# plai-group/latent-flexible-video-diffusion-modeling

Hardware: NVIDIA B200
Metric: denoiser frame-steps/sec (sampling) (higher is better)
Workload: dtype bf16

## Files before the change

latent-flexible-video-diffusion-modeling_b200/csrc/attn_temporal_tc.cu:

```cuda
#include "tc_common.cuh"
#include <mutex>

namespace fdm {

struct TtParams {
  const float* mask;
  __nv_bfloat16* b2;
  __nv_bfloat16* b3;
  __nv_bfloat16* P;
  __nv_bfloat16* out;
  float* attn_mean;
  int B, T, HW, C, F, heads;
  int TS;
  int Tn;
  int cf;
  int rows;
  int tmem_cols;
  float scale_log2e;
};

__device__ __forceinline__ uint64_t tt_desc_mn(uint32_t saddr) {
  uint64_t d = 0;
  d |= (uint64_t)((saddr & 0x3FFFF) >> 4);
  d |= (uint64_t)1 << 16;
  d |= (uint64_t)(1024 >> 4) << 32;
  d |= (uint64_t)1 << 46;
  d |= (uint64_t)2 << 61;
  return d;
}

__device__ __forceinline__ void tt_bulk_load(void* dst, const void* src, uint32_t bytes, uint64_t* bar) {
  asm volatile("cp.async.bulk.shared::cluster.global.mbarrier::complete_tx::bytes [%0], [%1], %2, [%3];"
               ::"r"(smem_u32(dst)), "l"(src), "r"(bytes), "r"(smem_u32(bar)) : "memory");
}

__device__ __forceinline__ uint32_t tt_pack(float a, float b) {
  __nv_bfloat162 v = __floats2bfloat162_rn(a, b);
  return *reinterpret_cast<uint32_t*>(&v);
}

template <class RowPtr>
__device__ __forceinline__ void tt_store_rows8(uint8_t* stage, int lane, const uint4 (&w)[4], RowPtr row_ptr, int np) {
#pragma unroll
  for (int q = 0; q < 4; ++q) *reinterpret_cast<uint4*>(stage + lane * 80 + q * 16) = w[q];
  __syncwarp();
  for (int idx = lane; idx < 32 * np; idx += 32) {
    const int row = idx / np, pc = idx - row * np;
    uint8_t* d = row_ptr(row);
    if (d != nullptr) *reinterpret_cast<uint2*>(d + pc * 8) = *reinterpret_cast<const uint2*>(stage + row * 80 + pc * 8);
  }
  __syncwarp();
}

__global__ void __launch_bounds__(128) rpe_bias_kernel(const __grid_constant__ CUtensorMap tq, const __grid_constant__ CUtensorMap trk,
                                                       const __grid_constant__ CUtensorMap trq, const TtParams p) {
  extern __shared__ uint8_t smem_raw[];
  uint8_t* smem = reinterpret_cast<uint8_t*>((reinterpret_cast<uintptr_t>(smem_raw) + 1023) & ~uintptr_t(1023));
  __shared__ __align__(8) uint64_t bar_load, bar_d;
  __shared__ uint32_t tmem_slot;
  const int tid = threadIdx.x, warp = tid >> 5;
  const int px0 = blockIdx.x * 128, j = blockIdx.y, bh = blockIdx.z;
  const int b = bh / p.heads, h = bh - b * p.heads;
  const int F = p.F, C = p.C, Tn = p.Tn;
  const int rtile = Tn * 128;
  uint8_t* q_s = smem;
  uint8_t* k_s = q_s + p.cf * 16384;
  uint8_t* rk_s = k_s + p.cf * 16384;
  uint8_t* rq_s = rk_s + p.cf * rtile;
  if (tid == 0) {
    asm volatile("prefetch.tensormap [%0];" ::"l"(&tq) : "memory");
    asm volatile("prefetch.tensormap [%0];" ::"l"(&trk) : "memory");
    asm volatile("prefetch.tensormap [%0];" ::"l"(&trq) : "memory");
    mbar_init(&bar_load, 1);
    mbar_init(&bar_d, 1);
    asm volatile("fence.mbarrier_init.release.cluster;" ::: "memory");
  }
  if (warp == 1) {
    asm volatile("tcgen05.alloc.cta_group::1.sync.aligned.shared::cta.b32 [%0], %1;" ::"r"(smem_u32(&tmem_slot)), "r"(p.tmem_cols));
    asm volatile("tcgen05.relinquish_alloc_permit.cta_group::1.sync.aligned;");
  }
  tcgen05_fence_before();
  __syncthreads();
  tcgen05_fence_after();
  const uint32_t tmem = tmem_slot;
  pdl_wait();
  if (tid == 0) {
    mbar_expect_tx(&bar_load, (uint32_t)(p.cf * (2 * p.rows * 128 + 2 * rtile)));
    for (int c = 0; c < p.cf; ++c) {
      const int ch = h * F + c * 64;
      tma_load_3d(q_s + c * 16384, &tq, &bar_load, ch, px0, b * p.T + j);
      tma_load_3d(k_s + c * 16384, &tq, &bar_load, C + ch, px0, b * p.T + j);
      tma_load_3d(rk_s + c * rtile, &trk, &bar_load, ch, 0, b * p.T + j);
      tma_load_3d(rq_s + c * rtile, &trq, &bar_load, ch, 0, b * p.T + j);
    }
    mbar_wait(&bar_load, 0);
    tcgen05_fence_after();
    const uint32_t idesc = make_idesc(Tn);
    const int ksteps = F / 16;
    for (int ks = 0; ks < ksteps; ++ks) {
      const int c = ks >> 2, kk = ks & 3;
      umma_bf16(tmem, make_smem_desc(smem_u32(q_s + c * 16384)) + 2 * kk, make_smem_desc(smem_u32(rk_s + c * rtile)) + 2 * kk, idesc, ks != 0);
    }
    for (int ks = 0; ks < ksteps; ++ks) {
      const int c = ks >> 2, kk = ks & 3;
      umma_bf16(tmem + Tn, make_smem_desc(smem_u32(k_s + c * 16384)) + 2 * kk, make_smem_desc(smem_u32(rq_s + c * rtile)) + 2 * kk, idesc, ks != 0);
    }
    umma_commit(&bar_d);
  }
  __syncwarp();
  mbar_wait(&bar_d, 0);
  tcgen05_fence_after();
  const uint32_t trow = tmem + ((uint32_t)(warp * 32) << 16);
  const int px = px0 + tid;
  const bool ok = tid < p.rows && px < p.HW;
  uint8_t* stage = smem + warp * 2560;
  const int lane = tid & 31;
  const int r0 = warp * 32;
  (void)ok;
  (void)px;
  for (int c0 = 0; c0 < Tn && c0 < p.TS; c0 += 32) {
    uint32_t v2[32], v3[32];
    {
      uint32_t a[16];
      tmem_ld_32x32b_x16(trow + c0, a);
#pragma unroll
      for (int k = 0; k < 16; ++k) v2[k] = a[k];
      tmem_ld_32x32b_x16(trow + Tn + c0, a);
#pragma unroll
      for (int k = 0; k < 16; ++k) v3[k] = a[k];
      if (c0 + 16 < Tn) {
        tmem_ld_32x32b_x16(trow + c0 + 16, a);
#pragma unroll
        for (int k = 0; k < 16; ++k) v2[16 + k] = a[k];
        tmem_ld_32x32b_x16(trow + Tn + c0 + 16, a);
#pragma unroll
        for (int k = 0; k < 16; ++k) v3[16 + k] = a[k];
      } else {
#pragma unroll
        for (int k = 0; k < 16; ++k) v2[16 + k] = v3[16 + k] = 0u;
      }
    }
    const int np = min(8, (p.TS - c0) / 4);
    auto rowp = [&](__nv_bfloat16* base, int r) -> uint8_t* {
      const int rr = r0 + r;
      if (rr >= p.rows || px0 + rr >= p.HW) return nullptr;
      return reinterpret_cast<uint8_t*>(base + (((size_t)bh * p.HW + px0 + rr) * p.T + j) * p.TS + c0);
    };
    uint4 w[4];
#pragma unroll
    for (int k = 0; k < 4; ++k)
      w[k] = make_uint4(tt_pack(__uint_as_float(v2[8 * k]), __uint_as_float(v2[8 * k + 1])), tt_pack(__uint_as_float(v2[8 * k + 2]), __uint_as_float(v2[8 * k + 3])),
                        tt_pack(__uint_as_float(v2[8 * k + 4]), __uint_as_float(v2[8 * k + 5])), tt_pack(__uint_as_float(v2[8 * k + 6]), __uint_as_float(v2[8 * k + 7])));
    if ((p.TS & 7) == 0) warp_store_rows64(stage, lane, w, [&](int r) { return rowp(p.b2, r); }, np >> 1);
    else tt_store_rows8(stage, lane, w, [&](int r) { return rowp(p.b2, r); }, np);
#pragma unroll
    for (int k = 0; k < 4; ++k)
      w[k] = make_uint4(tt_pack(__uint_as_float(v3[8 * k]), __uint_as_float(v3[8 * k + 1])), tt_pack(__uint_as_float(v3[8 * k + 2]), __uint_as_float(v3[8 * k + 3])),
                        tt_pack(__uint_as_float(v3[8 * k + 4]), __uint_as_float(v3[8 * k + 5])), tt_pack(__uint_as_float(v3[8 * k + 6]), __uint_as_float(v3[8 * k + 7])));
    if ((p.TS & 7) == 0) warp_store_rows64(stage, lane, w, [&](int r) { return rowp(p.b3, r); }, np >> 1);
    else tt_store_rows8(stage, lane, w, [&](int r) { return rowp(p.b3, r); }, np);
  }
  tcgen05_fence_before();
  __syncthreads();
  if (warp == 1) {
    tcgen05_fence_after();
    asm volatile("tcgen05.dealloc.cta_group::1.sync.aligned.b32 %0, %1;" ::"r"(tmem), "r"(p.tmem_cols));
  }
}

template <int TP>
__global__ void __launch_bounds__(128) attn_rows_kernel(const __grid_constant__ CUtensorMap tq4, const TtParams p) {
  constexpr int PL = 128 / TP;
  constexpr int W = TP < 32 ? 32 : TP;
  extern __shared__ uint8_t smem_raw[];
  uint8_t* smem = reinterpret_cast<uint8_t*>((reinterpret_cast<uintptr_t>(smem_raw) + 1023) & ~uintptr_t(1023));
  __shared__ __align__(8) uint64_t bar_load, bar_s, bar_o;
  __shared__ uint32_t tmem_slot;
  const int tid = threadIdx.x, warp = tid >> 5;
  const int px0 = blockIdx.x * PL, h = blockIdx.y, b = blockIdx.z;
  const int T = p.T, F = p.F, C = p.C, HW = p.HW;
  uint8_t* v_s = smem;
  uint8_t* q_s = v_s + p.cf * 16384;
  uint8_t* k_s = q_s + p.cf * 16384;
  uint8_t* p_s = q_s;
  if (tid == 0) {
    asm volatile("prefetch.tensormap [%0];" ::"l"(&tq4) : "memory");
    mbar_init(&bar_load, 1);
    mbar_init(&bar_s, 1);
    mbar_init(&bar_o, 1);
    asm volatile("fence.mbarrier_init.release.cluster;" ::: "memory");
  }
  if (warp == 1) {
    asm volatile("tcgen05.alloc.cta_group::1.sync.aligned.shared::cta.b32 [%0], %1;" ::"r"(smem_u32(&tmem_slot)), "r"(128));
    asm volatile("tcgen05.relinquish_alloc_permit.cta_group::1.sync.aligned;");
  }
  tcgen05_fence_before();
  __syncthreads();
  tcgen05_fence_after();
  const uint32_t tmem = tmem_slot;
  pdl_wait();
  const int bh = b * p.heads + h;
  const int TS = p.TS;
  __nv_bfloat16* b2_s = reinterpret_cast<__nv_bfloat16*>(smem + p.cf * 3 * 16384);
  __nv_bfloat16* b3_s = b2_s + PL * T * TS;
  if (tid == 0) {
    const uint32_t bias_bytes = (uint32_t)(PL * T * TS * sizeof(__nv_bfloat16));
    mbar_expect_tx(&bar_load, (uint32_t)(p.cf * 3 * 16384) + 2 * bias_bytes);
    for (int c = 0; c < p.cf; ++c) {
      const int ch = h * F + c * 64;
      tma_load_4d(q_s + c * 16384, &tq4, &bar_load, ch, 0, px0, b);
      tma_load_4d(k_s + c * 16384, &tq4, &bar_load, C + ch, 0, px0, b);
      tma_load_4d(v_s + c * 16384, &tq4, &bar_load, 2 * C + ch, 0, px0, b);
    }
    const size_t blk = ((size_t)bh * HW + px0) * T * TS;
    tt_bulk_load(b2_s, p.b2 + blk, bias_bytes, &bar_load);
    tt_bulk_load(b3_s, p.b3 + blk, bias_bytes, &bar_load);
    mbar_wait(&bar_load, 0);
    tcgen05_fence_after();
    const uint32_t idesc = make_idesc(128);
    const int ksteps = F / 16;
    for (int ks = 0; ks < ksteps; ++ks) {
      const int c = ks >> 2, kk = ks & 3;
      umma_bf16(tmem, make_smem_desc(smem_u32(q_s + c * 16384)) + 2 * kk, make_smem_desc(smem_u32(k_s + c * 16384)) + 2 * kk, idesc, ks != 0);
    }
    umma_commit(&bar_s);
  }
  __syncwarp();
  const int pl = tid / TP, t = tid - pl * TP;
  const int px = px0 + pl;
  const bool valid = t < T && px < HW;
  const int sub = TP < 32 ? (pl % (32 / TP)) : 0;
  const int col0 = (tid / W) * W;
  unsigned long long gbits = ~0ull;
  if (p.mask != nullptr) {
    const int lane = tid & 31;
    const float* maskb = p.mask + (size_t)b * T;
    const unsigned lo = __ballot_sync(0xffffffffu, lane < T && __ldg(maskb + lane) > 0.5f);
    const unsigned hi = __ballot_sync(0xffffffffu, lane + 32 < T && __ldg(maskb + lane + 32) > 0.5f);
    gbits = ((unsigned long long)hi << 32) | lo;
  }
  const bool grp = valid ? ((gbits >> t) & 1ull) != 0 : true;
  mbar_wait(&bar_load, 0);
  float bias[W];
  {
    float bt[TP];
    const __nv_bfloat16* b2r = b2_s + (size_t)(pl * T + (valid ? t : 0)) * TS;
    const __nv_bfloat16* b3col = b3_s + (size_t)pl * T * TS + (valid ? t : 0);
    auto fin = [&](int s, uint32_t bits) {
      const bool okj = valid && s < T && ((((gbits >> s) & 1ull) != 0) == grp);
      bt[s] = okj ? __uint_as_float(bits) + __bfloat162float(b3col[(size_t)(s < T ? s : 0) * TS]) : -INFINITY;
    };
    if ((TS & 7) == 0) {
#pragma unroll
      for (int k = 0; k < TP / 8; ++k) {
        uint4 r = make_uint4(0u, 0u, 0u, 0u);
        if (valid && 8 * k < T) r = reinterpret_cast<const uint4*>(b2r)[k];
        fin(8 * k, r.x << 16); fin(8 * k + 1, r.x & 0xffff0000u); fin(8 * k + 2, r.y << 16); fin(8 * k + 3, r.y & 0xffff0000u);
        fin(8 * k + 4, r.z << 16); fin(8 * k + 5, r.z & 0xffff0000u); fin(8 * k + 6, r.w << 16); fin(8 * k + 7, r.w & 0xffff0000u);
      }
    } else {
#pragma unroll
      for (int k = 0; k < TP / 4; ++k) {
        uint2 r = make_uint2(0u, 0u);
        if (valid && 4 * k < T) r = reinterpret_cast<const uint2*>(b2r)[k];
        fin(4 * k, r.x << 16); fin(4 * k + 1, r.x & 0xffff0000u); fin(4 * k + 2, r.y << 16); fin(4 * k + 3, r.y & 0xffff0000u);
      }
    }
#pragma unroll
    for (int j = 0; j < W; ++j) {
      const bool own = TP >= 32 ? true : ((j / TP) == sub);
      bias[j] = own ? bt[j % TP] : -INFINITY;
    }
  }
  __syncwarp();
  mbar_wait(&bar_s, 0);
  tcgen05_fence_after();

  const uint32_t trow = tmem + ((uint32_t)(warp * 32) << 16);
  float e[W];
  float mx = -INFINITY;
#pragma unroll
  for (int c = 0; c < W; c += 32) {
    uint32_t v[32];
    tmem_ld_32x32b_x32(trow + col0 + c, v);
#pragma unroll
    for (int j = 0; j < 32; ++j) {
      e[c + j] = (__uint_as_float(v[j]) + bias[c + j]) * p.scale_log2e;
      mx = fmaxf(mx, e[c + j]);
    }
  }
  float sum = 0.f;
#pragma unroll
  for (int j = 0; j < W; ++j) {
    e[j] = valid ? exp2f(e[j] - mx) : 0.f;
    sum += e[j];
  }
  const float inv = valid ? 1.f / sum : 0.f;
#pragma unroll
  for (int j = 0; j < W; ++j) e[j] *= inv;
  {
    const int sw = tid & 7;
    const int gp0 = col0 >> 3;
#pragma unroll
    for (int gp = 0; gp < 16; ++gp) {
      uint8_t* dst = p_s + (gp >> 3) * 16384 + tid * 128 + (((gp & 7) ^ sw) << 4);
      if (gp < gp0 || gp >= gp0 + W / 8) *reinterpret_cast<uint4*>(dst) = make_uint4(0u, 0u, 0u, 0u);
    }
#pragma unroll
    for (int q = 0; q < W / 8; ++q) {
      const int gp = gp0 + q;
      uint8_t* dst = p_s + (gp >> 3) * 16384 + tid * 128 + (((gp & 7) ^ sw) << 4);
      *reinterpret_cast<uint4*>(dst) = make_uint4(tt_pack(e[8 * q], e[8 * q + 1]), tt_pack(e[8 * q + 2], e[8 * q + 3]),
                                                  tt_pack(e[8 * q + 4], e[8 * q + 5]), tt_pack(e[8 * q + 6], e[8 * q + 7]));
    }
  }
  fence_proxy_async_smem();
  tcgen05_fence_before();
  __syncthreads();
  if (tid == 0) {
    tcgen05_fence_after();
    for (int c = 0; c < p.cf; ++c) {
      const int nf = min(64, F - c * 64);
      const uint32_t idesc = make_idesc(nf, 1);
      for (int ks = 0; ks < 8; ++ks)
        umma_bf16(tmem + c * 64, make_smem_desc(smem_u32(p_s + (ks >> 2) * 16384)) + 2 * (ks & 3),
                  tt_desc_mn(smem_u32(v_s + c * 16384 + ks * 2048)), idesc, ks != 0);
    }
    umma_commit(&bar_o);
  }
  const int lane = tid & 31;
  if (p.attn_mean != nullptr && valid) {
    float* arow = p.attn_mean + (((size_t)b * HW + px) * T + t) * T;
    const float hw_ = 1.f / (float)p.heads;
#pragma unroll
    for (int j = 0; j < W; ++j) {
      const bool own = TP >= 32 ? true : ((j / TP) == sub);
      if (own && (j % TP) < T) atomicAdd(arow + (j % TP), e[j] * hw_);
    }
  }
  {
    const int k = lane & 7;
#pragma unroll
    for (int i = 0; i < 8; ++i) {
      const int r = warp * 32 + i * 4 + (lane >> 3);
      const int rpl = r / TP, rt = r - rpl * TP;
      if (rt < T && px0 + rpl < HW) {
        uint4 val = make_uint4(0u, 0u, 0u, 0u);
        if (8 * k < TP) {
          const int gp = ((rpl * TP) >> 3) + k;
          val = *reinterpret_cast<const uint4*>(p_s + (gp >> 3) * 16384 + r * 128 + (((gp & 7) ^ (r & 7)) << 4));
        }
        *reinterpret_cast<uint4*>(reinterpret_cast<uint8_t*>(p.P + (((size_t)bh * HW + px0 + rpl) * T + rt) * 64) + k * 16) = val;
      }
    }
  }
  __syncwarp();
  mbar_wait(&bar_o, 0);
  tcgen05_fence_after();
  {
    uint8_t* stage = p_s + warp * 4096;
    for (int f = 0; f < F; f += 32) {
      uint32_t v[32];
      const bool two = f + 16 < F;
      {
        uint32_t a[16];
        tmem_ld_32x32b_x16(trow + f, a);
#pragma unroll
        for (int j = 0; j < 16; ++j) v[j] = a[j];
        if (two) {
          tmem_ld_32x32b_x16(trow + f + 16, a);
#pragma unroll
          for (int j = 0; j < 16; ++j) v[16 + j] = a[j];
        } else {
#pragma unroll
          for (int j = 0; j < 16; ++j) v[16 + j] = 0u;
        }
      }
      uint4 w[4];
#pragma unroll
      for (int k = 0; k < 4; ++k)
        w[k] = make_uint4(tt_pack(__uint_as_float(v[8 * k]), __uint_as_float(v[8 * k + 1])), tt_pack(__uint_as_float(v[8 * k + 2]), __uint_as_float(v[8 * k + 3])),
                          tt_pack(__uint_as_float(v[8 * k + 4]), __uint_as_float(v[8 * k + 5])), tt_pack(__uint_as_float(v[8 * k + 6]), __uint_as_float(v[8 * k + 7])));
      warp_store_rows64(stage, lane, w, [&](int rr) -> uint8_t* {
        const int r = warp * 32 + rr;
        const int rpl = r / TP, rt = r - rpl * TP;
        if (rt >= T || px0 + rpl >= HW) return nullptr;
        return reinterpret_cast<uint8_t*>(p.out + ((size_t)(b * T + rt) * HW + px0 + rpl) * C + h * F + f);
      }, two ? 4 : 2);
    }
  }
  tcgen05_fence_before();
  __syncthreads();
  if (warp == 1) {
    tcgen05_fence_after();
    asm volatile("tcgen05.dealloc.cta_group::1.sync.aligned.b32 %0, %1;" ::"r"(tmem), "r"(128));
  }
}

__global__ void __launch_bounds__(128) rpe_pv_kernel(const __grid_constant__ CUtensorMap tp4, const __grid_constant__ CUtensorMap trv,
                                                     const __grid_constant__ CUtensorMap to, const TtParams p) {
  extern __shared__ uint8_t smem_raw[];
  uint8_t* smem = reinterpret_cast<uint8_t*>((reinterpret_cast<uintptr_t>(smem_raw) + 1023) & ~uintptr_t(1023));
  __shared__ __align__(8) uint64_t bar_load, bar_d;
  __shared__ uint32_t tmem_slot;
  const int tid = threadIdx.x, warp = tid >> 5;
  const int px0 = blockIdx.x * 128, t = blockIdx.y, bh = blockIdx.z;
  const int b = bh / p.heads, h = bh - b * p.heads;
  const int F = p.F, Tn = p.Tn;
  const int rtile = Tn * 128;
  uint8_t* p_s = smem;
  uint8_t* rv_s = p_s + 16384;
  __nv_bfloat16* o_s = reinterpret_cast<__nv_bfloat16*>(rv_s + p.cf * rtile);
  if (tid == 0) {
    asm volatile("prefetch.tensormap [%0];" ::"l"(&tp4) : "memory");
    asm volatile("prefetch.tensormap [%0];" ::"l"(&trv) : "memory");
    asm volatile("prefetch.tensormap [%0];" ::"l"(&to) : "memory");
    mbar_init(&bar_load, 1);
    mbar_init(&bar_d, 1);
    asm volatile("fence.mbarrier_init.release.cluster;" ::: "memory");
  }
  if (warp == 1) {
    asm volatile("tcgen05.alloc.cta_group::1.sync.aligned.shared::cta.b32 [%0], %1;" ::"r"(smem_u32(&tmem_slot)), "r"(p.tmem_cols));
    asm volatile("tcgen05.relinquish_alloc_permit.cta_group::1.sync.aligned;");
  }
  tcgen05_fence_before();
  __syncthreads();
  tcgen05_fence_after();
  const uint32_t tmem = tmem_slot;
  pdl_wait();
  if (tid == 0) {
    mbar_expect_tx(&bar_load, (uint32_t)(p.rows * 128 + p.cf * rtile + p.rows * F * 2));
    tma_load_4d(p_s, &tp4, &bar_load, 0, t, px0, bh);
    tma_load_3d(o_s, &to, &bar_load, h * F, px0, b * p.T + t);
    for (int c = 0; c < p.cf; ++c) tma_load_3d(rv_s + c * rtile, &trv, &bar_load, h * F + c * 64, 0, b * p.T + t);
    mbar_wait(&bar_load, 0);
    tcgen05_fence_after();
    for (int c = 0; c < p.cf; ++c) {
      const int nf = min(64, F - c * 64);
      const uint32_t idesc = make_idesc(nf, 1);
      for (int ks = 0; ks < Tn / 16; ++ks)
        umma_bf16(tmem + c * 64, make_smem_desc(smem_u32(p_s)) + 2 * ks, tt_desc_mn(smem_u32(rv_s + c * rtile + ks * 2048)), idesc, ks != 0);
    }
    umma_commit(&bar_d);
  }
  __syncwarp();
  mbar_wait(&bar_d, 0);
  tcgen05_fence_after();
  const uint32_t trow = tmem + ((uint32_t)(warp * 32) << 16);
  const int px = px0 + tid;
  const bool ok = tid < p.rows && px < p.HW;
  const __nv_bfloat16* osrc = o_s + (size_t)(ok ? tid : 0) * F;
  uint8_t* stage = p_s + warp * 2560;
  const int lane = tid & 31;
  for (int f = 0; f < F; f += 32) {
    uint32_t v[32];
    const bool two = f + 16 < F;
    {
      uint32_t a[16];
      tmem_ld_32x32b_x16(trow + f, a);
#pragma unroll
      for (int j = 0; j < 16; ++j) v[j] = a[j];
      if (two) {
        tmem_ld_32x32b_x16(trow + f + 16, a);
#pragma unroll
        for (int j = 0; j < 16; ++j) v[16 + j] = a[j];
      } else {
#pragma unroll
        for (int j = 0; j < 16; ++j) v[16 + j] = 0u;
      }
    }
    uint4 w[4];
#pragma unroll
    for (int k = 0; k < 4; ++k) {
      uint4 o = make_uint4(0u, 0u, 0u, 0u);
      if (ok && (k < 2 || two)) o = *reinterpret_cast<const uint4*>(osrc + f + 8 * k);
      const uint32_t ow[4] = {o.x, o.y, o.z, o.w};
      uint32_t r[4];
#pragma unroll
      for (int q = 0; q < 4; ++q)
        r[q] = tt_pack(__uint_as_float(ow[q] << 16) + __uint_as_float(v[8 * k + 2 * q]),
                       __uint_as_float(ow[q] & 0xffff0000u) + __uint_as_float(v[8 * k + 2 * q + 1]));
      w[k] = make_uint4(r[0], r[1], r[2], r[3]);
    }
    warp_store_rows64(stage, lane, w, [&](int rr) -> uint8_t* {
      const int r = warp * 32 + rr;
      if (r >= p.rows || px0 + r >= p.HW) return nullptr;
      return reinterpret_cast<uint8_t*>(p.out + ((size_t)(b * p.T + t) * p.HW + px0 + r) * p.C + h * F + f);
    }, two ? 4 : 2);
  }
  tcgen05_fence_before();
  __syncthreads();
  if (warp == 1) {
    tcgen05_fence_after();
    asm volatile("tcgen05.dealloc.cta_group::1.sync.aligned.b32 %0, %1;" ::"r"(tmem), "r"(p.tmem_cols));
  }
}

static int tt_pow2(int v, int lo) {
  int r = lo;
  while (r < v) r <<= 1;
  return r;
}
static inline int tt_round_up(int v, int m) { return (v + m - 1) / m * m; }
int tt_row_stride(int T) {
  int t16 = tt_round_up(T, 8);
  if (((t16 / 8) & 1) == 0) t16 += 8;
  int t8 = tt_round_up(T, 4);
  if (((t8 / 4) & 1) == 0) t8 += 4;
  return t16 <= t8 ? t16 : t8;
}

static bool tt_shape_ok(const fdm_attn_temporal_args* a) {
  if (a->qkv_dtype != FDM_BF16 || a->out_dtype != FDM_BF16) return false;
  if (a->heads <= 0 || a->C % a->heads) return false;
  const int F = a->C / a->heads;
  if (F % 16 || F > 128 || a->C % 8) return false;
  if (a->T < 1 || a->T > 64) return false;
  const int TP = a->T <= 8 ? 8 : (a->T <= 16 ? 16 : (a->T <= 32 ? 32 : 64));
  if (a->HW % (128 / TP)) return false;
  return true;
}

size_t attn_temporal_tc_workspace(const fdm_attn_temporal_args* a) {
  if (!tt_shape_ok(a)) return 0;
  const size_t rows = (size_t)a->B * a->heads * a->HW * a->T;
  const size_t TS = tt_row_stride(a->T);
  return 2 * rows * TS * sizeof(__nv_bfloat16) + rows * 64 * sizeof(__nv_bfloat16);
}

template <typename Kern>
static int tt_set_smem(Kern k, int bytes) {
  cudaError_t e = cudaFuncSetAttribute(k, cudaFuncAttributeMaxDynamicSharedMemorySize, bytes);
  if (e != cudaSuccess) {
    set_last_error(e);
    return FDM_ERR_CUDA;
  }
  return FDM_OK;
}

static bool tt_encode(CUtensorMap* m, const void* ptr, int rank, const cuuint64_t* dims, const cuuint64_t* strides, const cuuint32_t* box) {
  EncodeTiledFn enc = get_tensormap_encoder();
  if (!enc) return false;
  cuuint32_t estr[4] = {1, 1, 1, 1};
  return enc(m, CU_TENSOR_MAP_DATA_TYPE_BFLOAT16, rank, const_cast<void*>(ptr), dims, strides, box, estr, CU_TENSOR_MAP_INTERLEAVE_NONE,
             CU_TENSOR_MAP_SWIZZLE_128B, CU_TENSOR_MAP_L2_PROMOTION_L2_128B, CU_TENSOR_MAP_FLOAT_OOB_FILL_NONE) == CUDA_SUCCESS;
}

int attn_temporal_tc_launch(const fdm_attn_temporal_args* a, cudaStream_t st) {
  if (!tt_shape_ok(a) || !a->Rq_op || !a->Rk_op || !a->Rv_op || !a->workspace) return FDM_ERR_UNSUPPORTED;
  const size_t need = attn_temporal_tc_workspace(a);
  FDM_REQUIRE((size_t)a->workspace_bytes >= need, FDM_ERR_BAD_ARG);
  const int B = a->B, T = a->T, HW = a->HW, C = a->C, heads = a->heads, F = C / heads;
  TtParams p;
  p.mask = a->mask;
  p.B = B; p.T = T; p.HW = HW; p.C = C; p.F = F; p.heads = heads;
  p.TS = tt_row_stride(T);
  p.Tn = tt_round_up(T, 16);
  p.cf = (F + 63) / 64;
  p.rows = HW < 128 ? HW : 128;
  p.scale_log2e = 1.4426950408889634f / sqrtf((float)F);
  const size_t rows = (size_t)B * heads * HW * T;
  p.b2 = reinterpret_cast<__nv_bfloat16*>(a->workspace);
  p.b3 = p.b2 + rows * p.TS;
  p.P = reinterpret_cast<__nv_bfloat16*>(p.b3 + rows * p.TS);
  p.out = reinterpret_cast<__nv_bfloat16*>(a->out);
  p.attn_mean = a->attn_mean;
  const int TP = T <= 8 ? 8 : (T <= 16 ? 16 : (T <= 32 ? 32 : 64));
  const int PL = 128 / TP;

  CUtensorMap tq3, tq4, trq, trk, trv, tp4;
  {
    cuuint64_t dims[3] = {(cuuint64_t)3 * C, (cuuint64_t)HW, (cuuint64_t)B * T};
    cuuint64_t strides[2] = {(cuuint64_t)3 * C * 2, (cuuint64_t)HW * 3 * C * 2};
    cuuint32_t box[3] = {64, (cuuint32_t)p.rows, 1};
    FDM_REQUIRE(tt_encode(&tq3, a->qkv, 3, dims, strides, box), FDM_ERR_UNSUPPORTED);
  }
  {
    cuuint64_t dims[4] = {(cuuint64_t)3 * C, (cuuint64_t)T, (cuuint64_t)HW, (cuuint64_t)B};
    cuuint64_t strides[3] = {(cuuint64_t)HW * 3 * C * 2, (cuuint64_t)3 * C * 2, (cuuint64_t)T * HW * 3 * C * 2};
    cuuint32_t box[4] = {64, (cuuint32_t)TP, (cuuint32_t)PL, 1};
    FDM_REQUIRE(tt_encode(&tq4, a->qkv, 4, dims, strides, box), FDM_ERR_UNSUPPORTED);
  }
  {
    cuuint64_t dims[3] = {(cuuint64_t)C, (cuuint64_t)T, (cuuint64_t)B * T};
    cuuint64_t strides[2] = {(cuuint64_t)C * 2, (cuuint64_t)T * C * 2};
    cuuint32_t box[3] = {64, (cuuint32_t)p.Tn, 1};
    FDM_REQUIRE(tt_encode(&trq, a->Rq_op, 3, dims, strides, box) && tt_encode(&trk, a->Rk_op, 3, dims, strides, box) &&
                    tt_encode(&trv, a->Rv_op, 3, dims, strides, box), FDM_ERR_UNSUPPORTED);
  }
  {
    cuuint64_t dims[4] = {64, (cuuint64_t)T, (cuuint64_t)HW, (cuuint64_t)B * heads};
    cuuint64_t strides[3] = {128, (cuuint64_t)T * 128, (cuuint64_t)HW * T * 128};
    cuuint32_t box[4] = {64, 1, (cuuint32_t)p.rows, 1};
    FDM_REQUIRE(tt_encode(&tp4, p.P, 4, dims, strides, box), FDM_ERR_UNSUPPORTED);
  }
  CUtensorMap to;
  {
    EncodeTiledFn enc = get_tensormap_encoder();
    cuuint64_t dims[3] = {(cuuint64_t)C, (cuuint64_t)HW, (cuuint64_t)B * T};
    cuuint64_t strides[2] = {(cuuint64_t)C * 2, (cuuint64_t)HW * C * 2};
    cuuint32_t box[3] = {(cuuint32_t)F, (cuuint32_t)p.rows, 1};
    cuuint32_t estr[3] = {1, 1, 1};
    FDM_REQUIRE(enc != nullptr && enc(&to, CU_TENSOR_MAP_DATA_TYPE_BFLOAT16, 3, a->out, dims, strides, box, estr, CU_TENSOR_MAP_INTERLEAVE_NONE,
                                      CU_TENSOR_MAP_SWIZZLE_NONE, CU_TENSOR_MAP_L2_PROMOTION_L2_128B,
                                      CU_TENSOR_MAP_FLOAT_OOB_FILL_NONE) == CUDA_SUCCESS, FDM_ERR_UNSUPPORTED);
  }
  const int smem1 = p.cf * (2 * 16384 + 2 * p.Tn * 128) + 1024;
  const int smem2 = p.cf * 3 * 16384 + 2 * PL * T * p.TS * (int)sizeof(__nv_bfloat16) + 1024;
  const int smem3 = 16384 + p.cf * p.Tn * 128 + p.rows * F * 2 + 1024;
  static std::once_flag once;
  static int attr_rc = FDM_OK;
  std::call_once(once, [] {
    int rc = tt_set_smem(rpe_bias_kernel, 100 * 1024);
    if (rc == FDM_OK) rc = tt_set_smem(attn_rows_kernel<8>, 200 * 1024);
    if (rc == FDM_OK) rc = tt_set_smem(attn_rows_kernel<16>, 200 * 1024);
    if (rc == FDM_OK) rc = tt_set_smem(attn_rows_kernel<32>, 200 * 1024);
    if (rc == FDM_OK) rc = tt_set_smem(attn_rows_kernel<64>, 200 * 1024);
    if (rc == FDM_OK) rc = tt_set_smem(rpe_pv_kernel, 100 * 1024);
    attr_rc = rc;
  });
  if (attr_rc != FDM_OK) return attr_rc;
  FDM_REQUIRE(smem1 <= 100 * 1024 && smem2 <= 200 * 1024 && smem3 <= 100 * 1024, FDM_ERR_UNSUPPORTED);

  TtParams p1 = p;
  p1.tmem_cols = tt_pow2(2 * p.Tn, 32);
  dim3 gridA((HW + 127) / 128, T, B * heads);
  fdm::launch(rpe_bias_kernel, gridA, dim3(128), smem1, st, tq3, trk, trq, p1);
  int rc = check_launch();
  if (rc != FDM_OK) return rc;
  dim3 gridB(HW / PL, heads, B);
  switch (TP) {
    case 8: fdm::launch(attn_rows_kernel<8>, gridB, dim3(128), smem2, st, tq4, p); break;
    case 16: fdm::launch(attn_rows_kernel<16>, gridB, dim3(128), smem2, st, tq4, p); break;
    case 32: fdm::launch(attn_rows_kernel<32>, gridB, dim3(128), smem2, st, tq4, p); break;
    default: fdm::launch(attn_rows_kernel<64>, gridB, dim3(128), smem2, st, tq4, p); break;
  }
  rc = check_launch();
  if (rc != FDM_OK) return rc;
  TtParams p3 = p;
  p3.tmem_cols = tt_pow2(F, 32);
  fdm::launch(rpe_pv_kernel, gridA, dim3(128), smem3, st, tp4, trv, to, p3);
  return check_launch();
}

}
```

Measured before the change: 94730.

## Pack temporal attention rows densely by T instead of padded power-of-two tiles

```diff
diff --git a/latent-flexible-video-diffusion-modeling_b200/csrc/attn_temporal_tc.cu b/latent-flexible-video-diffusion-modeling_b200/csrc/attn_temporal_tc.cu
--- a/latent-flexible-video-diffusion-modeling_b200/csrc/attn_temporal_tc.cu
+++ b/latent-flexible-video-diffusion-modeling_b200/csrc/attn_temporal_tc.cu
@@ -1,4 +1,5 @@
 #include "tc_common.cuh"
+#include <algorithm>
 #include <mutex>
 
 namespace fdm {
@@ -17,6 +18,11 @@
   int rows;
   int tmem_cols;
   float scale_log2e;
+  int v_stride;
+  int qk_row;
+  int qk_chunks;
+  int qk_stride;
+  int bias_cap;
 };
 
 __device__ __forceinline__ uint64_t tt_desc_mn(uint32_t saddr) {
@@ -26,6 +32,16 @@
   d |= (uint64_t)(1024 >> 4) << 32;
   d |= (uint64_t)1 << 46;
   d |= (uint64_t)2 << 61;
+  return d;
+}
+
+__device__ __forceinline__ uint64_t tt_desc_k64(uint32_t saddr) {
+  uint64_t d = 0;
+  d |= (uint64_t)((saddr & 0x3FFFF) >> 4);
+  d |= (uint64_t)1 << 16;
+  d |= (uint64_t)(512 >> 4) << 32;
+  d |= (uint64_t)1 << 46;
+  d |= (uint64_t)4 << 61;
   return d;
 }
 
@@ -168,23 +184,28 @@
   }
 }
 
-template <int TP>
-__global__ void __launch_bounds__(128) attn_rows_kernel(const __grid_constant__ CUtensorMap tq4, const TtParams p) {
-  constexpr int PL = 128 / TP;
-  constexpr int W = TP < 32 ? 32 : TP;
+template <int NC>
+__global__ void __launch_bounds__(128, NC <= 4 ? 4 : 2) attn_rows_kernel(const __grid_constant__ CUtensorMap tqk4, const __grid_constant__ CUtensorMap tv4,
+                                                        const TtParams p) {
   extern __shared__ uint8_t smem_raw[];
   uint8_t* smem = reinterpret_cast<uint8_t*>((reinterpret_cast<uintptr_t>(smem_raw) + 1023) & ~uintptr_t(1023));
   __shared__ __align__(8) uint64_t bar_load, bar_s, bar_o;
   __shared__ uint32_t tmem_slot;
-  const int tid = threadIdx.x, warp = tid >> 5;
+  const int tid = threadIdx.x, warp = tid >> 5, lane = tid & 31;
+  const int T = p.T, F = p.F, C = p.C, HW = p.HW, TS = p.TS;
+  const int PL = 128 / T, R = PL * T;
   const int px0 = blockIdx.x * PL, h = blockIdx.y, b = blockIdx.z;
-  const int T = p.T, F = p.F, C = p.C, HW = p.HW;
+  const int bh = b * p.heads + h;
   uint8_t* v_s = smem;
-  uint8_t* q_s = v_s + p.cf * 16384;
-  uint8_t* k_s = q_s + p.cf * 16384;
+  uint8_t* q_s = v_s + p.cf * p.v_stride;
+  uint8_t* k_s = q_s + p.qk_chunks * p.qk_stride;
+  uint8_t* b2_raw = k_s + p.qk_chunks * p.qk_stride;
+  uint8_t* b3_raw = b2_raw + p.bias_cap;
   uint8_t* p_s = q_s;
+  const bool p_over_bias = q_s + 32768 > b2_raw;
   if (tid == 0) {
-    asm volatile("prefetch.tensormap [%0];" ::"l"(&tq4) : "memory");
+    asm volatile("prefetch.tensormap [%0];" ::"l"(&tqk4) : "memory");
+    asm volatile("prefetch.tensormap [%0];" ::"l"(&tv4) : "memory");
     mbar_init(&bar_load, 1);
     mbar_init(&bar_s, 1);
     mbar_init(&bar_o, 1);
@@ -199,119 +220,130 @@
   tcgen05_fence_after();
   const uint32_t tmem = tmem_slot;
   pdl_wait();
-  const int bh = b * p.heads + h;
-  const int TS = p.TS;
-  __nv_bfloat16* b2_s = reinterpret_cast<__nv_bfloat16*>(smem + p.cf * 3 * 16384);
-  __nv_bfloat16* b3_s = b2_s + PL * T * TS;
+  const int npx = min(PL, HW - px0);
+  const size_t blk = ((size_t)bh * HW + px0) * T * TS;
+  const uint8_t* b2_g = reinterpret_cast<const uint8_t*>(p.b2 + blk);
+  const uint8_t* b3_g = reinterpret_cast<const uint8_t*>(p.b3 + blk);
+  const uint32_t d2 = (uint32_t)reinterpret_cast<uintptr_t>(b2_g) & 15u, d3 = (uint32_t)reinterpret_cast<uintptr_t>(b3_g) & 15u;
+  const __nv_bfloat16* b2_s = reinterpret_cast<const __nv_bfloat16*>(b2_raw + d2);
+  const __nv_bfloat16* b3_s = reinterpret_cast<const __nv_bfloat16*>(b3_raw + d3);
   if (tid == 0) {
-    const uint32_t bias_bytes = (uint32_t)(PL * T * TS * sizeof(__nv_bfloat16));
-    mbar_expect_tx(&bar_load, (uint32_t)(p.cf * 3 * 16384) + 2 * bias_bytes);
-    for (int c = 0; c < p.cf; ++c) {
+    const uint32_t bias_bytes = (uint32_t)(npx * T * TS) * (uint32_t)sizeof(__nv_bfloat16);
+    const uint32_t n2 = (d2 + bias_bytes + 15u) & ~15u, n3 = (d3 + bias_bytes + 15u) & ~15u;
+    mbar_expect_tx(&bar_load, (uint32_t)(R * (2 * p.qk_chunks * p.qk_row + p.cf * 128)) + n2 + n3);
+    for (int c = 0; c < p.qk_chunks; ++c) {
       const int ch = h * F + c * 64;
-      tma_load_4d(q_s + c * 16384, &tq4, &bar_load, ch, 0, px0, b);
-      tma_load_4d(k_s + c * 16384, &tq4, &bar_load, C + ch, 0, px0, b);
-      tma_load_4d(v_s + c * 16384, &tq4, &bar_load, 2 * C + ch, 0, px0, b);
-    }
-    const size_t blk = ((size_t)bh * HW + px0) * T * TS;
-    tt_bulk_load(b2_s, p.b2 + blk, bias_bytes, &bar_load);
-    tt_bulk_load(b3_s, p.b3 + blk, bias_bytes, &bar_load);
+      tma_load_4d(q_s + c * p.qk_stride, &tqk4, &bar_load, ch, 0, px0, b);
+      tma_load_4d(k_s + c * p.qk_stride, &tqk4, &bar_load, C + ch, 0, px0, b);
+    }
+    for (int c = 0; c < p.cf; ++c) tma_load_4d(v_s + c * p.v_stride, &tv4, &bar_load, 2 * C + h * F + c * 64, 0, px0, b);
+    tt_bulk_load(b2_raw, b2_g - d2, n2, &bar_load);
+    tt_bulk_load(b3_raw, b3_g - d3, n3, &bar_load);
     mbar_wait(&bar_load, 0);
     tcgen05_fence_after();
     const uint32_t idesc = make_idesc(128);
     const int ksteps = F / 16;
     for (int ks = 0; ks < ksteps; ++ks) {
-      const int c = ks >> 2, kk = ks & 3;
-      umma_bf16(tmem, make_smem_desc(smem_u32(q_s + c * 16384)) + 2 * kk, make_smem_desc(smem_u32(k_s + c * 16384)) + 2 * kk, idesc, ks != 0);
+      if (p.qk_row == 64) {
+        umma_bf16(tmem, tt_desc_k64(smem_u32(q_s)) + 2 * ks, tt_desc_k64(smem_u32(k_s)) + 2 * ks, idesc, ks != 0);
+      } else {
+        const int c = ks >> 2, kk = ks & 3;
+        umma_bf16(tmem, make_smem_desc(smem_u32(q_s + c * p.qk_stride)) + 2 * kk, make_smem_desc(smem_u32(k_s + c * p.qk_stride)) + 2 * kk,
+                  idesc, ks != 0);
+      }
     }
     umma_commit(&bar_s);
   }
   __syncwarp();
-  const int pl = tid / TP, t = tid - pl * TP;
-  const int px = px0 + pl;
-  const bool valid = t < T && px < HW;
-  const int sub = TP < 32 ? (pl % (32 / TP)) : 0;
-  const int col0 = (tid / W) * W;
+  for (int r = R + tid; r < p.v_stride / 128; r += 128)
+    for (int c = 0; c < p.cf; ++c)
+#pragma unroll
+      for (int q = 0; q < 8; ++q) *reinterpret_cast<uint4*>(v_s + c * p.v_stride + r * 128 + q * 16) = make_uint4(0u, 0u, 0u, 0u);
+  const int pl = tid / T, t = tid - pl * T;
+  const int ob = pl * T;
+  const bool valid = tid < R && px0 + pl < HW;
   unsigned long long gbits = ~0ull;
   if (p.mask != nullptr) {
-    const int lane = tid & 31;
     const float* maskb = p.mask + (size_t)b * T;
     const unsigned lo = __ballot_sync(0xffffffffu, lane < T && __ldg(maskb + lane) > 0.5f);
     const unsigned hi = __ballot_sync(0xffffffffu, lane + 32 < T && __ldg(maskb + lane + 32) > 0.5f);
     gbits = ((unsigned long long)hi << 32) | lo;
   }
   const bool grp = valid ? ((gbits >> t) & 1ull) != 0 : true;
+  const bool wrows = warp * 32 < R;
+  const int c_lo = wrows ? (warp * 32 / T) * T / 16 * 16 : 0;
+  const int c_hi = wrows ? (min(warp * 32 + 31, R - 1) / T + 1) * T : 0;
+  const int c_end = c_lo + (c_hi - c_lo + 15) / 16 * 16;
   mbar_wait(&bar_load, 0);
-  float bias[W];
-  {
-    float bt[TP];
-    const __nv_bfloat16* b2r = b2_s + (size_t)(pl * T + (valid ? t : 0)) * TS;
-    const __nv_bfloat16* b3col = b3_s + (size_t)pl * T * TS + (valid ? t : 0);
-    auto fin = [&](int s, uint32_t bits) {
-      const bool okj = valid && s < T && ((((gbits >> s) & 1ull) != 0) == grp);
-      bt[s] = okj ? __uint_as_float(bits) + __bfloat162float(b3col[(size_t)(s < T ? s : 0) * TS]) : -INFINITY;
-    };
-    if ((TS & 7) == 0) {
-#pragma unroll
-      for (int k = 0; k < TP / 8; ++k) {
-        uint4 r = make_uint4(0u, 0u, 0u, 0u);
-        if (valid && 8 * k < T) r = reinterpret_cast<const uint4*>(b2r)[k];
-        fin(8 * k, r.x << 16); fin(8 * k + 1, r.x & 0xffff0000u); fin(8 * k + 2, r.y << 16); fin(8 * k + 3, r.y & 0xffff0000u);
-        fin(8 * k + 4, r.z << 16); fin(8 * k + 5, r.z & 0xffff0000u); fin(8 * k + 6, r.w << 16); fin(8 * k + 7, r.w & 0xffff0000u);
-      }
-    } else {
-#pragma unroll
-      for (int k = 0; k < TP / 4; ++k) {
-        uint2 r = make_uint2(0u, 0u);
-        if (valid && 4 * k < T) r = reinterpret_cast<const uint2*>(b2r)[k];
-        fin(4 * k, r.x << 16); fin(4 * k + 1, r.x & 0xffff0000u); fin(4 * k + 2, r.y << 16); fin(4 * k + 3, r.y & 0xffff0000u);
-      }
-    }
-#pragma unroll
-    for (int j = 0; j < W; ++j) {
-      const bool own = TP >= 32 ? true : ((j / TP) == sub);
-      bias[j] = own ? bt[j % TP] : -INFINITY;
-    }
-  }
-  __syncwarp();
   mbar_wait(&bar_s, 0);
   tcgen05_fence_after();
 
   const uint32_t trow = tmem + ((uint32_t)(warp * 32) << 16);
-  float e[W];
+  const __nv_bfloat16* b2r = b2_s + (size_t)(valid ? tid : 0) * TS;
+  const __nv_bfloat16* b3c = b3_s + (size_t)(valid ? ob : 0) * TS + (valid ? t : 0);
+  const unsigned long long gsame = grp ? gbits : ~gbits;
+  float x[NC * 16];
   float mx = -INFINITY;
 #pragma unroll
-  for (int c = 0; c < W; c += 32) {
-    uint32_t v[32];
-    tmem_ld_32x32b_x32(trow + col0 + c, v);
-#pragma unroll
-    for (int j = 0; j < 32; ++j) {
-      e[c + j] = (__uint_as_float(v[j]) + bias[c + j]) * p.scale_log2e;
-      mx = fmaxf(mx, e[c + j]);
-    }
-  }
+  for (int cc = 0; cc < NC; ++cc) {
+    const int c = c_lo + cc * 16;
+    if (c < c_hi) {
+      uint32_t v[16];
+      tmem_ld_32x32b_x16(trow + c, v);
+#pragma unroll
+      for (int j = 0; j < 16; ++j) {
+        const int s = c + j - ob;
+        const bool own = valid && (unsigned)s < (unsigned)T && ((gsame >> (s & 63)) & 1ull) != 0;
+        const int sc = own ? s : 0;
+        const float bias = __bfloat162float(b2r[sc]) + __bfloat162float(b3c[sc * TS]);
+        x[cc * 16 + j] = own ? (__uint_as_float(v[j]) + bias) * p.scale_log2e : -INFINITY;
+        mx = fmaxf(mx, x[cc * 16 + j]);
+      }
+    } else {
+#pragma unroll
+      for (int j = 0; j < 16; ++j) x[cc * 16 + j] = -INFINITY;
+    }
+  }
+  if (!valid) mx = 0.f;
   float sum = 0.f;
 #pragma unroll
-  for (int j = 0; j < W; ++j) {
-    e[j] = valid ? exp2f(e[j] - mx) : 0.f;
-    sum += e[j];
+  for (int j = 0; j < NC * 16; ++j) {
+    x[j] = exp2f(x[j] - mx);
+    sum += x[j];
   }
   const float inv = valid ? 1.f / sum : 0.f;
-#pragma unroll
-  for (int j = 0; j < W; ++j) e[j] *= inv;
+  if (p_over_bias) __syncthreads();
   {
     const int sw = tid & 7;
-    const int gp0 = col0 >> 3;
 #pragma unroll
     for (int gp = 0; gp < 16; ++gp) {
-      uint8_t* dst = p_s + (gp >> 3) * 16384 + tid * 128 + (((gp & 7) ^ sw) << 4);
-      if (gp < gp0 || gp >= gp0 + W / 8) *reinterpret_cast<uint4*>(dst) = make_uint4(0u, 0u, 0u, 0u);
-    }
-#pragma unroll
-    for (int q = 0; q < W / 8; ++q) {
-      const int gp = gp0 + q;
-      uint8_t* dst = p_s + (gp >> 3) * 16384 + tid * 128 + (((gp & 7) ^ sw) << 4);
-      *reinterpret_cast<uint4*>(dst) = make_uint4(tt_pack(e[8 * q], e[8 * q + 1]), tt_pack(e[8 * q + 2], e[8 * q + 3]),
-                                                  tt_pack(e[8 * q + 4], e[8 * q + 5]), tt_pack(e[8 * q + 6], e[8 * q + 7]));
+      if (gp < (c_lo >> 3) || gp >= (c_end >> 3))
+        *reinterpret_cast<uint4*>(p_s + (gp >> 3) * 16384 + tid * 128 + (((gp & 7) ^ sw) << 4)) = make_uint4(0u, 0u, 0u, 0u);
+    }
+#pragma unroll
+    for (int j = 0; j < NC * 16; ++j) x[j] *= inv;
+#pragma unroll
+    for (int cc = 0; cc < NC; ++cc) {
+      const int c = c_lo + cc * 16;
+      if (c < c_hi) {
+        const float* e = x + cc * 16;
+#pragma unroll
+        for (int q = 0; q < 2; ++q) {
+          const int gp = (c >> 3) + q;
+          *reinterpret_cast<uint4*>(p_s + (gp >> 3) * 16384 + tid * 128 + (((gp & 7) ^ sw) << 4)) =
+              make_uint4(tt_pack(e[8 * q], e[8 * q + 1]), tt_pack(e[8 * q + 2], e[8 * q + 3]), tt_pack(e[8 * q + 4], e[8 * q + 5]),
+                         tt_pack(e[8 * q + 6], e[8 * q + 7]));
+        }
+      }
+    }
+    if (p.attn_mean != nullptr && valid) {
+      float* arow = p.attn_mean + (((size_t)b * HW + px0 + pl) * T + t) * T;
+      const float hw_ = 1.f / (float)p.heads;
+#pragma unroll
+      for (int j = 0; j < NC * 16; ++j) {
+        const int s = c_lo + j - ob;
+        if (c_lo + j < c_hi && (unsigned)s < (unsigned)T) atomicAdd(arow + s, x[j] * hw_);
+      }
     }
   }
   fence_proxy_async_smem();
@@ -322,35 +354,39 @@
     for (int c = 0; c < p.cf; ++c) {
       const int nf = min(64, F - c * 64);
       const uint32_t idesc = make_idesc(nf, 1);
-      for (int ks = 0; ks < 8; ++ks)
+      for (int ks = 0; ks * 16 < R; ++ks)
         umma_bf16(tmem + c * 64, make_smem_desc(smem_u32(p_s + (ks >> 2) * 16384)) + 2 * (ks & 3),
-                  tt_desc_mn(smem_u32(v_s + c * 16384 + ks * 2048)), idesc, ks != 0);
+                  tt_desc_mn(smem_u32(v_s + c * p.v_stride + ks * 2048)), idesc, ks != 0);
     }
     umma_commit(&bar_o);
   }
-  const int lane = tid & 31;
-  if (p.attn_mean != nullptr && valid) {
-    float* arow = p.attn_mean + (((size_t)b * HW + px) * T + t) * T;
-    const float hw_ = 1.f / (float)p.heads;
-#pragma unroll
-    for (int j = 0; j < W; ++j) {
-      const bool own = TP >= 32 ? true : ((j / TP) == sub);
-      if (own && (j % TP) < T) atomicAdd(arow + (j % TP), e[j] * hw_);
-    }
-  }
   {
     const int k = lane & 7;
-#pragma unroll
+#pragma unroll 1
     for (int i = 0; i < 8; ++i) {
       const int r = warp * 32 + i * 4 + (lane >> 3);
-      const int rpl = r / TP, rt = r - rpl * TP;
-      if (rt < T && px0 + rpl < HW) {
-        uint4 val = make_uint4(0u, 0u, 0u, 0u);
-        if (8 * k < TP) {
-          const int gp = ((rpl * TP) >> 3) + k;
-          val = *reinterpret_cast<const uint4*>(p_s + (gp >> 3) * 16384 + r * 128 + (((gp & 7) ^ (r & 7)) << 4));
+      const int rpl = r / T, rt = r - rpl * T;
+      if (r < R && px0 + rpl < HW) {
+        uint32_t o[4] = {0u, 0u, 0u, 0u};
+        const int nv = T - 8 * k;
+        if (nv > 0) {
+          const int col = rpl * T + 8 * k, gp = col >> 3, sh = col & 7;
+          auto piece = [&](int g) { return *reinterpret_cast<const uint4*>(p_s + (g >> 3) * 16384 + r * 128 + (((g & 7) ^ (r & 7)) << 4)); };
+          const uint4 a = piece(gp);
+          const uint4 c = (sh != 0 && gp + 1 < 16) ? piece(gp + 1) : make_uint4(0u, 0u, 0u, 0u);
+          const uint32_t w[8] = {a.x, a.y, a.z, a.w, c.x, c.y, c.z, c.w};
+          const int q = sh >> 1;
+          uint32_t x[5];
+#pragma unroll
+          for (int j = 0; j < 5; ++j) x[j] = q == 0 ? w[j] : q == 1 ? w[j + 1] : q == 2 ? w[j + 2] : w[j + 3];
+#pragma unroll
+          for (int j = 0; j < 4; ++j) {
+            const uint32_t v = __funnelshift_r(x[j], x[j + 1], 16 * (sh & 1));
+            o[j] = 2 * j + 1 < nv ? v : (2 * j < nv ? (v & 0xffffu) : 0u);
+          }
         }
-        *reinterpret_cast<uint4*>(reinterpret_cast<uint8_t*>(p.P + (((size_t)bh * HW + px0 + rpl) * T + rt) * 64) + k * 16) = val;
+        *reinterpret_cast<uint4*>(reinterpret_cast<uint8_t*>(p.P + (((size_t)bh * HW + px0 + rpl) * T + rt) * 64) + k * 16) =
+            make_uint4(o[0], o[1], o[2], o[3]);
       }
     }
   }
@@ -383,8 +419,8 @@
                           tt_pack(__uint_as_float(v[8 * k + 4]), __uint_as_float(v[8 * k + 5])), tt_pack(__uint_as_float(v[8 * k + 6]), __uint_as_float(v[8 * k + 7])));
       warp_store_rows64(stage, lane, w, [&](int rr) -> uint8_t* {
         const int r = warp * 32 + rr;
-        const int rpl = r / TP, rt = r - rpl * TP;
-        if (rt >= T || px0 + rpl >= HW) return nullptr;
+        const int rpl = r / T, rt = r - rpl * T;
+        if (r >= R || px0 + rpl >= HW) return nullptr;
         return reinterpret_cast<uint8_t*>(p.out + ((size_t)(b * T + rt) * HW + px0 + rpl) * C + h * F + f);
       }, two ? 4 : 2);
     }
@@ -502,6 +538,15 @@
   return r;
 }
 static inline int tt_round_up(int v, int m) { return (v + m - 1) / m * m; }
+static int tt_window_chunks(int T) {
+  const int PL = 128 / T, R = PL * T;
+  int m = 0;
+  for (int w = 0; w * 32 < R; ++w) {
+    const int lo = (w * 32 / T) * T / 16 * 16, hi = (std::min(w * 32 + 31, R - 1) / T + 1) * T;
+    m = std::max(m, (hi - lo + 15) / 16);
+  }
+  return m;
+}
 int tt_row_stride(int T) {
   int t16 = tt_round_up(T, 8);
   if (((t16 / 8) & 1) == 0) t16 += 8;
@@ -516,8 +561,6 @@
   const int F = a->C / a->heads;
   if (F % 16 || F > 128 || a->C % 8) return false;
   if (a->T < 1 || a->T > 64) return false;
-  const int TP = a->T <= 8 ? 8 : (a->T <= 16 ? 16 : (a->T <= 32 ? 32 : 64));
-  if (a->HW % (128 / TP)) return false;
   return true;
 }
 
@@ -538,12 +581,13 @@
   return FDM_OK;
 }
 
-static bool tt_encode(CUtensorMap* m, const void* ptr, int rank, const cuuint64_t* dims, const cuuint64_t* strides, const cuuint32_t* box) {
+static bool tt_encode(CUtensorMap* m, const void* ptr, int rank, const cuuint64_t* dims, const cuuint64_t* strides, const cuuint32_t* box,
+                      CUtensorMapSwizzle swz = CU_TENSOR_MAP_SWIZZLE_128B) {
   EncodeTiledFn enc = get_tensormap_encoder();
   if (!enc) return false;
   cuuint32_t estr[4] = {1, 1, 1, 1};
   return enc(m, CU_TENSOR_MAP_DATA_TYPE_BFLOAT16, rank, const_cast<void*>(ptr), dims, strides, box, estr, CU_TENSOR_MAP_INTERLEAVE_NONE,
-             CU_TENSOR_MAP_SWIZZLE_128B, CU_TENSOR_MAP_L2_PROMOTION_L2_128B, CU_TENSOR_MAP_FLOAT_OOB_FILL_NONE) == CUDA_SUCCESS;
+             swz, CU_TENSOR_MAP_L2_PROMOTION_L2_128B, CU_TENSOR_MAP_FLOAT_OOB_FILL_NONE) == CUDA_SUCCESS;
 }
 
 int attn_temporal_tc_launch(const fdm_attn_temporal_args* a, cudaStream_t st) {
@@ -565,10 +609,14 @@
   p.P = reinterpret_cast<__nv_bfloat16*>(p.b3 + rows * p.TS);
   p.out = reinterpret_cast<__nv_bfloat16*>(a->out);
   p.attn_mean = a->attn_mean;
-  const int TP = T <= 8 ? 8 : (T <= 16 ? 16 : (T <= 32 ? 32 : 64));
-  const int PL = 128 / TP;
-
-  CUtensorMap tq3, tq4, trq, trk, trv, tp4;
+  const int PL = 128 / T, R = PL * T, R8 = tt_round_up(R, 8);
+  p.v_stride = p.cf == 1 ? R8 * 128 : 16384;
+  p.qk_row = F <= 32 ? 64 : 128;
+  p.qk_chunks = F <= 32 ? 1 : p.cf;
+  p.qk_stride = R8 * p.qk_row;
+  p.bias_cap = tt_round_up(PL * T * p.TS * (int)sizeof(__nv_bfloat16), 16) + 16;
+
+  CUtensorMap tq3, tqk4, tv4, trq, trk, trv, tp4;
   {
     cuuint64_t dims[3] = {(cuuint64_t)3 * C, (cuuint64_t)HW, (cuuint64_t)B * T};
     cuuint64_t strides[2] = {(cuuint64_t)3 * C * 2, (cuuint64_t)HW * 3 * C * 2};
@@ -578,8 +626,11 @@
   {
     cuuint64_t dims[4] = {(cuuint64_t)3 * C, (cuuint64_t)T, (cuuint64_t)HW, (cuuint64_t)B};
     cuuint64_t strides[3] = {(cuuint64_t)HW * 3 * C * 2, (cuuint64_t)3 * C * 2, (cuuint64_t)T * HW * 3 * C * 2};
-    cuuint32_t box[4] = {64, (cuuint32_t)TP, (cuuint32_t)PL, 1};
-    FDM_REQUIRE(tt_encode(&tq4, a->qkv, 4, dims, strides, box), FDM_ERR_UNSUPPORTED);
+    cuuint32_t box[4] = {64, (cuuint32_t)T, (cuuint32_t)PL, 1};
+    FDM_REQUIRE(tt_encode(&tv4, a->qkv, 4, dims, strides, box), FDM_ERR_UNSUPPORTED);
+    box[0] = (cuuint32_t)p.qk_row / 2;
+    FDM_REQUIRE(tt_encode(&tqk4, a->qkv, 4, dims, strides, box, p.qk_row == 64 ? CU_TENSOR_MAP_SWIZZLE_64B : CU_TENSOR_MAP_SWIZZLE_128B),
+                FDM_ERR_UNSUPPORTED);
   }
   {
     cuuint64_t dims[3] = {(cuuint64_t)C, (cuuint64_t)T, (cuuint64_t)B * T};
@@ -606,16 +657,15 @@
                                       CU_TENSOR_MAP_FLOAT_OOB_FILL_NONE) == CUDA_SUCCESS, FDM_ERR_UNSUPPORTED);
   }
   const int smem1 = p.cf * (2 * 16384 + 2 * p.Tn * 128) + 1024;
-  const int smem2 = p.cf * 3 * 16384 + 2 * PL * T * p.TS * (int)sizeof(__nv_bfloat16) + 1024;
+  const int qkb_end = p.cf * p.v_stride + 2 * p.qk_chunks * p.qk_stride + 2 * p.bias_cap;
+  const int smem2 = std::max(qkb_end, p.cf * p.v_stride + 32768) + 1024;
   const int smem3 = 16384 + p.cf * p.Tn * 128 + p.rows * F * 2 + 1024;
   static std::once_flag once;
   static int attr_rc = FDM_OK;
   std::call_once(once, [] {
     int rc = tt_set_smem(rpe_bias_kernel, 100 * 1024);
+    if (rc == FDM_OK) rc = tt_set_smem(attn_rows_kernel<4>, 200 * 1024);
     if (rc == FDM_OK) rc = tt_set_smem(attn_rows_kernel<8>, 200 * 1024);
-    if (rc == FDM_OK) rc = tt_set_smem(attn_rows_kernel<16>, 200 * 1024);
-    if (rc == FDM_OK) rc = tt_set_smem(attn_rows_kernel<32>, 200 * 1024);
-    if (rc == FDM_OK) rc = tt_set_smem(attn_rows_kernel<64>, 200 * 1024);
     if (rc == FDM_OK) rc = tt_set_smem(rpe_pv_kernel, 100 * 1024);
     attr_rc = rc;
   });
@@ -628,13 +678,9 @@
   fdm::launch(rpe_bias_kernel, gridA, dim3(128), smem1, st, tq3, trk, trq, p1);
   int rc = check_launch();
   if (rc != FDM_OK) return rc;
-  dim3 gridB(HW / PL, heads, B);
-  switch (TP) {
-    case 8: fdm::launch(attn_rows_kernel<8>, gridB, dim3(128), smem2, st, tq4, p); break;
-    case 16: fdm::launch(attn_rows_kernel<16>, gridB, dim3(128), smem2, st, tq4, p); break;
-    case 32: fdm::launch(attn_rows_kernel<32>, gridB, dim3(128), smem2, st, tq4, p); break;
-    default: fdm::launch(attn_rows_kernel<64>, gridB, dim3(128), smem2, st, tq4, p); break;
-  }
+  dim3 gridB((HW + PL - 1) / PL, heads, B);
+  if (tt_window_chunks(T) <= 4) fdm::launch(attn_rows_kernel<4>, gridB, dim3(128), smem2, st, tqk4, tv4, p);
+  else fdm::launch(attn_rows_kernel<8>, gridB, dim3(128), smem2, st, tqk4, tv4, p);
   rc = check_launch();
   if (rc != FDM_OK) return rc;
   TtParams p3 = p;
```

Result: slower. 91370, median of 6 (-3.5%).
